# someone-in-somewhere/multimodal_rag

Hardware: AMD Instinct MI355X
Metric: chunks embedded/sec + queries/sec top_k=5 over 1M×768 at 1/2/4/8 GPUs (higher is better)
Workload: dtype f16

## Files before the change

### include/mmrag.h

```cpp
#ifndef MMRAG_H
#define MMRAG_H

#include <stddef.h>
#include <stdint.h>

#ifdef __cplusplus
extern "C" {
#endif

#define MMRAG_OK 0
#define MMRAG_EINVAL 1
#define MMRAG_EWORKSPACE 2
#define MMRAG_EHIP 3
#define MMRAG_EUNSUPPORTED 4

#define MMRAG_F32 0
#define MMRAG_F16 1
#define MMRAG_BF16 2
#define MMRAG_F8E4M3 3

#define MMRAG_MAX_K 20

int mmrag_abi_version(void);
const char *mmrag_last_error(void);

int64_t mmrag_padded_dim(int d, int dtype);

size_t mmrag_cosine_topk_workspace_bytes(int B, int64_t n, int k);

int mmrag_cosine_topk(const void *q, const void *corpus, int B, int64_t n, int d, int64_t ld,
                      int dtype, int k, int64_t row_offset, const uint32_t *alive_bits,
                      float *out_scores, int64_t *out_rows, void *workspace,
                      size_t workspace_bytes, void *stream);

int mmrag_cosine_topk_lists(const void *q, const void *corpus, int B, int64_t n, int d, int64_t ld,
                            int dtype, int k, const uint32_t *alive_bits, void *workspace,
                            size_t workspace_bytes, void *stream);
int mmrag_cosine_topk_select(int B, int64_t n, int k, int64_t row_offset, const void *workspace,
                             float *out_scores, int64_t *out_rows, void *stream);

#define MMRAG_MAX_K_DEEP 4096
size_t mmrag_cosine_topk_deep_workspace_bytes(int B, int64_t n, int k);
int mmrag_cosine_topk_deep(const void *q, const void *corpus, int B, int64_t n, int d, int64_t ld,
                           int dtype, int k, int64_t row_offset, const uint32_t *alive_bits,
                           float *out_scores, int64_t *out_rows, void *workspace,
                           size_t workspace_bytes, void *stream);

#define MMRAG_MAX_RESCORE_CANDIDATES 4096
int mmrag_rescore_topk(const void *q, const void *plane, int64_t ld, int dtype, int d, const int64_t *cand_rows,
                       int B, int C, int k, float *out_scores, int64_t *out_rows, void *stream);

int mmrag_merge_topk(const float *scores, const int64_t *rows, int G, int B, int k_in, int k,
                     float *out_scores, int64_t *out_rows, void *stream);
int mmrag_merge_topk_host(const float *scores, const int64_t *rows, int G, int B, int k_in,
                          int k, float *out_scores, int64_t *out_rows);
int mmrag_merge_topk_host_packed(const void *blocks, int G, int B, int k_in, int k,
                                 float *out_scores, int64_t *out_rows);

int mmrag_append_rows(void *corpus, int64_t capacity, int64_t ld, int dtype, int64_t n_used,
                      const float *new_rows, int64_t m, int d, void *stream);

int mmrag_gather_rows(void *dst, const void *src, int64_t ld, int dtype,
                      const int64_t *keep_rows, int64_t m, void *stream);

int mmrag_fetch_rows_f32(const void *corpus, int64_t ld, int dtype, const int64_t *rows,
                         int64_t m, int d, float *out, void *stream);

int mmrag_copy_to_host_async(void *dst_host, const void *src_dev, size_t bytes, void *stream);


#define MMRAG_ACT_NONE 0
#define MMRAG_ACT_GELU 1
// ... 191 lines not shown
```

### multimodal_rag_amd/_native.py

```python
from __future__ import annotations

import ctypes
import os
import threading
from ctypes import c_char_p, c_float, c_int, c_int32, c_int64, c_size_t, c_void_p
from typing import Optional, Tuple

import numpy as np
import torch

_PKG = os.path.dirname(os.path.abspath(__file__))
LIB_PATH = os.path.join(_PKG, "lib", "libmmrag.so")

F32, F16, BF16, F8E4M3 = 0, 1, 2, 3
MAX_K = 20
MAX_K_DEEP = 4096
MAX_MMR_CANDIDATES = 1024
MAX_RESCORE_CANDIDATES = 4096
MAX_GROUP_CANDIDATES, MAX_GROUPS, MAX_GROUP_SIZE = 4096, 256, 16
MAX_FUSE_LISTS, MAX_FUSE_CANDIDATES, MAX_FUSE_RESULTS = 16, 256, 4096
FUSE_METHODS = {"rrf": 0, "max": 1}
MAX_JOIN_PAIRS = 1 << 26
MAX_CLUSTERS = 4096
MAX_SCOPE_GROUPS = 64
MAX_RELATED_ROWS, MAX_RELATED_SETS = 8192, 64
MAX_RECOMMEND_EXAMPLES = 16
MAX_LATE_QUERY_TOKENS, MAX_LATE_DOC_TOKENS = 128, 512
MAX_LATE_PAIRS = 65535
_DT2TORCH = {F32: torch.float32, F16: torch.float16, BF16: torch.bfloat16, F8E4M3: torch.float8_e4m3fn}
_TORCH2DT = {v: k for k, v in _DT2TORCH.items()}

_lib = None
_lock = threading.Lock()


class MMRagNativeError(RuntimeError):
    pass


def _declare(lib):
    lib.mmrag_abi_version.restype = c_int
    lib.mmrag_last_error.restype = c_char_p
    lib.mmrag_padded_dim.restype = c_int64
    lib.mmrag_padded_dim.argtypes = [c_int, c_int]
    lib.mmrag_cosine_topk_workspace_bytes.restype = c_size_t
    lib.mmrag_cosine_topk_workspace_bytes.argtypes = [c_int, c_int64, c_int]
    lib.mmrag_cosine_topk.restype = c_int
    lib.mmrag_cosine_topk.argtypes = [c_void_p, c_void_p, c_int, c_int64, c_int, c_int64, c_int, c_int,
                                      c_int64, c_void_p, c_void_p, c_void_p, c_void_p, c_size_t, c_void_p]
    lib.mmrag_cosine_topk_lists.restype = c_int
    lib.mmrag_cosine_topk_lists.argtypes = [c_void_p, c_void_p, c_int, c_int64, c_int, c_int64, c_int, c_int,
                                            c_void_p, c_void_p, c_size_t, c_void_p]
    lib.mmrag_internal_search_uses_qs.restype = c_int
    lib.mmrag_internal_search_uses_qs.argtypes = [c_int, c_int64, c_int64, c_int, c_int]
    lib.mmrag_internal_cosine_topk_lists_ex.restype = c_int
    lib.mmrag_internal_cosine_topk_lists_ex.argtypes = [c_void_p, c_void_p, c_int, c_int64, c_int, c_int64, c_int,
                                                        c_int, c_void_p, c_void_p, c_size_t, c_void_p, ctypes.c_uint]
    lib.mmrag_cosine_topk_select.restype = c_int
    lib.mmrag_cosine_topk_select.argtypes = [c_int, c_int64, c_int, c_int64, c_void_p, c_void_p, c_void_p, c_void_p]
    lib.mmrag_cosine_topk_deep_workspace_bytes.restype = c_size_t
    lib.mmrag_cosine_topk_deep_workspace_bytes.argtypes = [c_int, c_int64, c_int]
    lib.mmrag_cosine_topk_deep.restype = c_int
    lib.mmrag_cosine_topk_deep.argtypes = lib.mmrag_cosine_topk.argtypes
    lib.mmrag_internal_cosine_topk_deep_ex.restype = c_int
    lib.mmrag_internal_cosine_topk_deep_ex.argtypes = lib.mmrag_cosine_topk.argtypes + [ctypes.c_uint, c_int64]
    lib.mmrag_rescore_topk.restype = c_int
    lib.mmrag_rescore_topk.argtypes = [c_void_p, c_void_p, c_int64, c_int, c_int, c_void_p, c_int, c_int, c_int,
                                       c_void_p, c_void_p, c_void_p]
    lib.mmrag_merge_topk.restype = c_int
    lib.mmrag_merge_topk.argtypes = [c_void_p, c_void_p, c_int, c_int, c_int, c_int, c_void_p, c_void_p, c_void_p]
    lib.mmrag_merge_topk_host.restype = c_int
    lib.mmrag_merge_topk_host.argtypes = [c_void_p, c_void_p, c_int, c_int, c_int, c_int, c_void_p, c_void_p]
    lib.mmrag_merge_topk_host_packed.restype = c_int
    lib.mmrag_merge_topk_host_packed.argtypes = [c_void_p, c_int, c_int, c_int, c_int, c_void_p, c_void_p]
    lib.mmrag_append_rows.restype = c_int
    lib.mmrag_append_rows.argtypes = [c_void_p, c_int64, c_int64, c_int, c_int64, c_void_p, c_int64, c_int, c_void_p]
    lib.mmrag_gather_rows.restype = c_int
    lib.mmrag_gather_rows.argtypes = [c_void_p, c_void_p, c_int64, c_int, c_void_p, c_int64, c_void_p]
    lib.mmrag_fetch_rows_f32.restype = c_int
    lib.mmrag_fetch_rows_f32.argtypes = [c_void_p, c_int64, c_int, c_void_p, c_int64, c_int, c_void_p, c_void_p]
    lib.mmrag_device_info.restype = c_int
    lib.mmrag_device_info.argtypes = [ctypes.POINTER(c_int), ctypes.POINTER(c_int), ctypes.POINTER(c_int64)]
    lib.mmrag_bench_stream_copy.restype = c_int
    lib.mmrag_bench_stream_copy.argtypes = [c_void_p, c_void_p, c_int64, c_void_p]
    lib.mmrag_bench_mfma_f16.restype = c_int
# ... 204 lines not shown
        raise MMRagNativeError(f"{who}: q and {other} must be contiguous 2-D tensors")
    if q.dtype != rows.dtype or q.shape[1] != rows.shape[1]:
        raise MMRagNativeError(f"{who}: q and {other} must share dtype and padded width")
    if n is not None and n > rows.shape[0]:
        raise MMRagNativeError(f"{who}: n={n} exceeds corpus capacity {rows.shape[0]}")


def _topk_out(B: int, k: int, device, packed: bool = False) -> Tuple[torch.Tensor, torch.Tensor]:
    if not packed:
        return (torch.empty((B, k), dtype=torch.float32, device=device),
                torch.empty((B, k), dtype=torch.int64, device=device))
    buf = torch.empty(B * k * 12, dtype=torch.uint8, device=device)
    return buf[B * k * 8:].view(torch.float32).view(B, k), buf[: B * k * 8].view(torch.int64).view(B, k)


def search_uses_query_stationary(B: int, n: int, d: int, k: int, dtype: torch.dtype) -> bool:
    return bool(lib().mmrag_internal_search_uses_qs(B, n, padded_dim(d, dtype), _TORCH2DT[dtype], k))


def search_kernel_name(B: int, n: int, d: int, k: int, dtype: torch.dtype) -> str:
    v = lib().mmrag_internal_search_uses_qs(B, n, padded_dim(d, dtype), _TORCH2DT[dtype], k)
    return {0: "cosine_topk_kernel (slab-ring)", 1: "cosine_topk_qs_kernel", 2: "cosine_topk_walk_kernel"}[v]


def padded_dim(d: int, dtype: torch.dtype) -> int:
    v = lib().mmrag_padded_dim(int(d), _TORCH2DT[dtype])
    if v < 0:
        raise MMRagNativeError(f"padded_dim: bad arguments d={d} dtype={dtype}")
    return int(v)


DBG_NO_PREPASS, DBG_8_WAVES, DBG_NO_QS, DBG_FORCE_QS = 1, 2, 4, 8
DBG_OLD_QS, DBG_MFMA32, DBG_MFMA16, DBG_NO_DYN, DBG_NO_SEED = 0x10000, 0x20000, 0x40000, 0x80000, 0x100000


def cosine_topk(q: torch.Tensor, corpus: torch.Tensor, n: int, d: int, k: int, row_offset: int = 0,
                alive_bits: Optional[torch.Tensor] = None,
                workspace: Optional[torch.Tensor] = None, dbg: int = 0,
                packed_out: bool = False) -> Tuple[torch.Tensor, torch.Tensor]:
    _dev_check(q, corpus, alive_bits)
    _check_q_rows("cosine_topk", q, corpus, n)
    B, ld = q.shape
    L = lib()
    need = L.mmrag_cosine_topk_workspace_bytes(B, n, k)
    if workspace is None or _nbytes(workspace) < need:
        workspace = torch.empty(max(need, 16), dtype=torch.uint8, device=q.device)
    out_s, out_r = _topk_out(B, k, q.device, packed_out)
    if dbg:
        cosine_topk_lists(q, corpus, n, d, k, workspace, alive_bits=alive_bits, dbg=dbg)
        return cosine_topk_select(B, n, k, row_offset, workspace, out_s, out_r)
    with torch.cuda.device(q.device):
        st = L.mmrag_cosine_topk(q.data_ptr(), corpus.data_ptr(), B, n, d, ld, _TORCH2DT[q.dtype], k, row_offset,
                                 alive_bits.data_ptr() if alive_bits is not None else None,
                                 out_s.data_ptr(), out_r.data_ptr(), workspace.data_ptr(), _nbytes(workspace),
                                 _stream_ptr(q.device))
    _check(st, "mmrag_cosine_topk")
    return out_s, out_r


DEEP_DBG_NO_BOUND = 1


def cosine_topk_deep(q: torch.Tensor, corpus: torch.Tensor, n: int, d: int, k: int, row_offset: int = 0,
                     alive_bits: Optional[torch.Tensor] = None, workspace: Optional[torch.Tensor] = None,
                     dbg: int = 0, cap: int = 0) -> Tuple[torch.Tensor, torch.Tensor]:
    _dev_check(q, corpus, alive_bits)
# ... 1127 lines not shown
        st = lib().mmrag_resize_crop_u8(src.data_ptr(), H, W, src.stride(0), bx.data_ptr(), kx.data_ptr(),
                                        int(kx.shape[1]), by.data_ptr(), ky.data_ptr(), int(ky.shape[1]), out_h, out_w,
                                        y_lo, y_hi, tmp.data_ptr(), out.data_ptr(), _stream_ptr(src.device))
    _check(st, "mmrag_resize_crop_u8")
    return out


def copy_to_host_async(dst_host: torch.Tensor, src_dev: torch.Tensor, stream: int) -> None:
    nbytes = src_dev.numel() * src_dev.element_size()
    if dst_host.is_cuda or not src_dev.is_cuda or dst_host.numel() * dst_host.element_size() < nbytes:
        raise MMRagNativeError("copy_to_host_async: need a host destination at least as large as the device source")
    _check(lib().mmrag_copy_to_host_async(dst_host.data_ptr(), src_dev.data_ptr(), nbytes, stream),
           "mmrag_copy_to_host_async")


class SearchPlan:

    def __init__(self, q: torch.Tensor, corpus: torch.Tensor, n: int, d: int, k: int, workspace: torch.Tensor,
                 alive_bits: Optional[torch.Tensor] = None):
        _dev_check(q, corpus, workspace, alive_bits)
        if q.dtype != corpus.dtype or q.shape[1] != corpus.shape[1] or not q.is_contiguous() or not corpus.is_contiguous():
            raise MMRagNativeError("SearchPlan: q and corpus must be contiguous and share dtype and padded width")
        if n > corpus.shape[0]:
            raise MMRagNativeError(f"SearchPlan: n={n} exceeds corpus capacity {corpus.shape[0]}")
        need = lib().mmrag_cosine_topk_workspace_bytes(q.shape[0], n, k)
        if _nbytes(workspace) < need:
            raise MMRagNativeError("SearchPlan: workspace too small")
        self._keep = (q, corpus, workspace, alive_bits)
        self.B, self.n, self.k = q.shape[0], n, k
        self._scan_args = (q.data_ptr(), corpus.data_ptr(), q.shape[0], n, d, q.shape[1], _TORCH2DT[q.dtype], k,
                           alive_bits.data_ptr() if alive_bits is not None else None, workspace.data_ptr(),
                           _nbytes(workspace))
        self._ws = workspace.data_ptr()
        self._scan = lib().mmrag_cosine_topk_lists
        self._select = lib().mmrag_cosine_topk_select

    def scan(self, stream: int) -> None:
        st = self._scan(*self._scan_args, stream)
        if st:
            _check(st, "mmrag_cosine_topk_lists")

    def select(self, row_offset: int, out_scores_ptr: int, out_rows_ptr: int, stream: int) -> None:
        st = self._select(self.B, self.n, self.k, row_offset, self._ws, out_scores_ptr, out_rows_ptr, stream)
        if st:
            _check(st, "mmrag_cosine_topk_select")
```

### multimodal_rag_amd/csrc/search.hip

```cpp
#include "slab_ring.h"

#include <stdlib.h>

using namespace mmrag;

namespace mmrag_impl {

template <int DT, int WN, int K, int NSTAGE, int NW, bool SEEDED>
__global__ __launch_bounds__(64 * NW, NW / 4) void cosine_topk_kernel(const KParams p) {
#if defined(__HIP_DEVICE_COMPILE__)
#include "slab_ring_body.inc"
#endif
}

template <int K>
struct FullList {
    float v[K];
    long long r[K];
    __device__ inline void init() {
#pragma unroll
        for (int i = 0; i < K; ++i) {
            v[i] = NEG_INF;
            r[i] = LLONG_MAX;
        }
    }
    __device__ inline void insert(float x, long long xr) {
#pragma unroll
        for (int j = 0; j < K; ++j) {
            const bool b = better(x, xr, v[j], r[j]);
            const float nv = b ? x : v[j];
            const float nx = b ? v[j] : x;
            const long long nr = b ? xr : r[j];
            const long long nxr = b ? r[j] : xr;
            v[j] = nv;
            x = nx;
// ... 83 lines not shown
                    out_r[(size_t)q * k_out + i] = valid ? orr[i] + row_offset : -1;
                }
            }
            if (thr0 != nullptr) {
                const bool full = orr[K - 1] != LLONG_MAX && ov[K - 1] > NEG_INF;
                thr0[q] = full ? ov[K - 1] : NEG_INF;
#pragma unroll
                for (int i = 0; i < K; ++i) {
                    const bool valid = orr[i] != LLONG_MAX && ov[i] > NEG_INF;
                    seed_s[(size_t)q * seed_q_stride + i] = valid ? ov[i] : NEG_INF;
                    seed_r[(size_t)q * seed_q_stride + i] = valid ? (int)orr[i] : INT_MAX;
                }
            }
        }
    }
}

struct Plan {
    int K;
    int WN;
    int NW;
    int grid_x, grid_y;
    int n_tiles;
    int n_lists;
    int b_pad;
    int pre_tiles;
    bool qs_ok;
    bool qs_room;
};

constexpr unsigned DBG_NO_PREPASS = 1u, DBG_8_WAVES = 2u, DBG_NO_QS = 4u, DBG_FORCE_QS = 8u;
constexpr unsigned DBG_OLD_QS = 0x10000u, DBG_MFMA32 = 0x20000u, DBG_MFMA16 = 0x40000u, DBG_NO_DYN = 0x80000u,
                   DBG_NO_SEED = 0x100000u;

Plan make_plan(int B, long long n, int k, unsigned dbg = 0) {
    Plan pl;
    pl.K = k <= 5 ? 5 : (k <= 10 ? 10 : 20);
    pl.WN = plan_wn(B);
    const int qrows = 32 * pl.WN;
    pl.grid_y = (B + qrows - 1) / qrows;
    pl.n_tiles = (int)((n + TM - 1) / TM);
    const int cus = num_cus();
    pl.grid_x = plan_walkers(pl.n_tiles, pl.grid_y);
    pl.NW = (pl.K == 5 && pl.WN == 8 && !(dbg & DBG_8_WAVES)) ? 16 : 8;
    pl.pre_tiles = 0;
    const bool want_pre = (pl.WN == 8 || pl.K > 5) && pl.n_tiles >= 3 * cus;
    if (want_pre && !(dbg & DBG_NO_PREPASS)) pl.pre_tiles = cus;
    pl.n_lists = pl.grid_x + (want_pre ? 1 : 0);
    pl.b_pad = pl.grid_y * qrows;
    pl.qs_room = pl.WN == 8 && pl.n_tiles >= cus;
    const bool long_enough = pl.K <= 5 ? pl.n_tiles * 4 >= 15 * cus : pl.n_tiles >= 6 * cus;
    pl.qs_ok = pl.qs_room && !(dbg & DBG_NO_QS) && (long_enough || (dbg & DBG_FORCE_QS));
    return pl;
}

template <int DT, int WN, int K, int NSTAGE, int NW = 8, bool SEEDED = false>
void launch_main(const KParams &p, dim3 grid, hipStream_t s) {
    KParams kp = p;
    kp.walkers = (int)grid.x;
    kp.share_l2 = grid.y > 1;
    cosine_topk_kernel<DT, WN, K, NSTAGE, NW, SEEDED><<<grid.x * grid.y, 64 * NW, 0, s>>>(kp);
}

template <int DT, int K>
void dispatch_deep(const Plan &pl, const KParams &p, dim3 grid, hipStream_t s) {
    if (pl.WN == 2) launch_main<DT, 2, K, 3>(p, grid, s);
// ... 64 lines not shown
__global__ void fill_seed_empty_kernel(float *s, int *r, long long q_stride, int K, long long n_queries) {
    const long long q = (long long)blockIdx.x * blockDim.x + threadIdx.x;
    if (q < n_queries)
        for (int i = 0; i < K; ++i) {
            s[q * q_stride + i] = NEG_INF;
            r[q * q_stride + i] = INT_MAX;
        }
}

int check_search_args(const char *name, int k_max, const void *q, const void *corpus, int B, int64_t n, int d, int64_t ld,
                      int dtype, int k) {
    MMRAG_CHECK_ARG(dtype >= 0 && dtype <= MMRAG_F8E4M3, "%s: bad dtype %d", name, dtype);
    MMRAG_CHECK_ARG(B > 0, "%s: B must be positive (got %d)", name, B);
    MMRAG_CHECK_ARG(k >= 1 && k <= k_max, "%s: k=%d outside 1..%d", name, k, k_max);
    MMRAG_CHECK_ARG(n >= 0 && n < (int64_t)INT_MAX - TM, "%s: n=%lld out of range", name, (long long)n);
    MMRAG_CHECK_ARG(d > 0 && ld >= d, "%s: need 0 < d <= ld (d=%d ld=%lld)", name, d, (long long)ld);
    const int64_t row_bytes = ld * esize(dtype);
    MMRAG_CHECK_ARG(row_bytes % SLAB == 0, "%s: row bytes %lld not a multiple of %d (use mmrag_padded_dim)", name,
                    (long long)row_bytes, SLAB);
    MMRAG_CHECK_ARG(row_bytes * TM < (int64_t)UINT_MAX, "%s: rows too long", name);
    MMRAG_CHECK_ARG(q, "%s: null q", name);
    MMRAG_CHECK_ARG(n == 0 || corpus, "%s: null corpus", name);
    MMRAG_CHECK_ARG(((uintptr_t)q % 16) == 0 && ((uintptr_t)corpus % 16) == 0, "%s: q/corpus must be 16-byte aligned",
                    name);
    return MMRAG_OK;
}

}
using namespace mmrag_impl;

extern "C" {

struct WsLayout {
    size_t entries, off_r, off_thr, off_ts, off_tr, off_cnt, cnt_bytes, off_pub, off_pthr, off_tk, xch_end, total;
};
static WsLayout ws_layout(const Plan &pl) {
    WsLayout w;
    w.entries = (size_t)pl.b_pad * pl.n_lists * pl.K;
    w.off_r = w.entries * sizeof(float);
    w.off_thr = w.off_r + w.entries * sizeof(int);
    w.off_ts = w.off_thr + (size_t)pl.b_pad * sizeof(float);
    w.off_tr = (w.off_ts + (size_t)pl.b_pad * pl.K * sizeof(float) + 15) / 16 * 16;
    w.off_cnt = (w.off_tr + (size_t)pl.b_pad * pl.K * sizeof(long long) + 63) / 64 * 64;
    w.cnt_bytes = 0;
    w.off_pub = w.off_cnt + w.cnt_bytes;
    w.off_pthr = w.off_pub + (pl.qs_room ? (size_t)pl.b_pad * pl.grid_x * sizeof(float) : 0);
    w.off_tk = w.off_pthr + (pl.qs_room ? (size_t)pl.b_pad * sizeof(float) : 0);
    w.xch_end = w.off_tk + (pl.qs_room ? ((size_t)pl.grid_y * sizeof(unsigned) + 63) / 64 * 64 : 0);
    w.total = w.xch_end;
    return w;
}

size_t mmrag_cosine_topk_workspace_bytes(int B, int64_t n, int k) {
    if (B <= 0 || n < 0 || k < 1 || k > MMRAG_MAX_K) return 0;
    return ws_layout(make_plan(B, n, k)).total + 256;
}

int mmrag_internal_cosine_topk_lists_ex(const void *q, const void *corpus, int B, int64_t n, int d, int64_t ld,
                                        int dtype, int k, const uint32_t *alive_bits, void *workspace,
                                        size_t workspace_bytes, void *stream, unsigned dbg) {
    if (int st = check_search_args("cosine_topk", MMRAG_MAX_K, q, corpus, B, n, d, ld, dtype, k)) return st;
    if (n == 0) return MMRAG_OK;
    const Plan pl = make_plan(B, n, k, dbg);
    const WsLayout wl = ws_layout(pl);
    if (!workspace || workspace_bytes < wl.total) {
        set_error("cosine_topk: workspace %zu bytes < required %zu", workspace_bytes, wl.total);
        return MMRAG_EWORKSPACE;
    }
    MMRAG_CHECK_ARG(((uintptr_t)workspace % 16) == 0, "cosine_topk: workspace must be 16-byte aligned");

    KParams p;
    p.q = (const char *)q;
    p.corpus = (const char *)corpus;
    p.alive_bits = alive_bits;
    p.cand_s = (float *)workspace;
    p.cand_r = (int *)((char *)workspace + wl.off_r);
    p.n = n;
    p.B = B;
    p.row_bytes = (unsigned)(ld * esize(dtype));
    p.n_tiles = pl.n_tiles;
    p.n_lists = pl.n_lists;
    p.tile0 = 0;
    p.thr0 = nullptr;
    p.dbg = dbg;
    p.stamps = ((dbg & DBG_QS_CLOCK) && workspace_bytes >= wl.total + 256 * (size_t)(pl.grid_x * pl.grid_y)) ? (unsigned long long *)((char *)workspace + wl.total) : nullptr;
    p.walkers = pl.grid_x;
    p.share_l2 = pl.grid_y > 1;
    p.sample_best = nullptr;
    p.pub_best = nullptr;
    p.pub_thr = nullptr;
    p.tickets = nullptr;
    p.p_static = INT_MAX / 2;
    hipStream_t s = (hipStream_t)stream;
    const size_t seed_off = (size_t)(pl.n_lists - 1) * pl.K;
    const int walk_mfma = (dbg & DBG_MFMA32) ? 32 : ((dbg & DBG_MFMA16) ? 16 : (pl.K == 5 ? QSW_DEFAULT_MFMA : 32));
    if (pl.qs_ok && !(dbg & DBG_OLD_QS) && qsw_supported(dtype, p.row_bytes, pl.K, walk_mfma)) {
        const int tiles = (int)((n + QS_TILE_ROWS - 1) / QS_TILE_ROWS);
        const int per = tiles / pl.grid_x;
        p.n_tiles = tiles;
        p.pub_best = nullptr;
        p.pub_thr = nullptr;
        p.tickets = nullptr;
        p.p_static = INT_MAX / 2;
        const bool seed = per >= 12 && !(dbg & DBG_NO_SEED);
        const bool dyn = pl.grid_y == 1 && per >= 24 && !(dbg & DBG_NO_DYN);
        if (seed || dyn) {
            MMRAG_CHECK_HIP(hipMemsetD32Async((hipDeviceptr_t)((char *)workspace + wl.off_pub), (int)TICKET0,
                                              (wl.xch_end - wl.off_pub) / 4, s));
            if (seed) {
                p.pub_best = (float *)((char *)workspace + wl.off_pub);
                p.pub_thr = (float *)((char *)workspace + wl.off_pthr);
            }
            if (dyn) {
                p.tickets = (unsigned *)((char *)workspace + wl.off_tk);
                const int tail = per / 10 > 3 ? per / 10 : 3;
                p.p_static = per - tail;
            }
        }
        if (int st = qsw_launch(dtype, pl.K, walk_mfma, p, pl.grid_x, pl.grid_y, s)) return st;
        MMRAG_CHECK_HIP(hipGetLastError());
        return MMRAG_OK;
    }
    if (pl.qs_ok && qs_supported(dtype, p.row_bytes, pl.K)) {
        const int tiles = (int)((n + QS_TILE_ROWS - 1) / QS_TILE_ROWS);
        float *thr0 = nullptr;
        if (pl.pre_tiles > 0) {
            KParams ks = p;
            ks.n_tiles = pl.pre_tiles * (TM / QS_TILE_ROWS);
            ks.sample_best = (float *)((char *)workspace + wl.off_pub);
            if (int st = qs_launch(dtype, pl.K, ks, pl.grid_x, pl.grid_y, s)) return st;
            thr0 = (float *)((char *)workspace + wl.off_thr);
            if (int st = qs_seed_thresholds(pl.K, ks.sample_best, pl.grid_x, pl.b_pad, thr0, s)) return st;
        }
        p.n_tiles = tiles;
        p.thr0 = thr0;
        if (int st = qs_launch(dtype, pl.K, p, pl.grid_x, pl.grid_y, s)) return st;
        MMRAG_CHECK_HIP(hipGetLastError());
        return MMRAG_OK;
    }
    auto run = [&](int tile0, int n_tiles, int grid_x, const float *thr0) -> int {
        KParams kp = p;
// ... 16 lines not shown
        const long long n_cand = (long long)pre_grid * pl.K;
        launch_merge<int>(pl.K, p.cand_s, p.cand_r, n_cand, n_cand, 0, (long long)pl.n_lists * pl.K, B, pl.K, 0, top_s,
                          top_r, s, thr0, p.cand_s + seed_off, p.cand_r + seed_off, (long long)pl.n_lists * pl.K);
        MMRAG_CHECK_HIP(hipGetLastError());
        if (int st = run(pre, pl.n_tiles - pre, pl.grid_x, thr0)) return st;
    } else {
        if (pl.n_lists > pl.grid_x) {
            const long long total = (long long)pl.b_pad;
            fill_seed_empty_kernel<<<(unsigned)((total + 255) / 256), 256, 0, s>>>(
                p.cand_s + seed_off, p.cand_r + seed_off, (long long)pl.n_lists * pl.K, pl.K, total);
        }
        if (int st = run(0, pl.n_tiles, pl.grid_x, nullptr)) return st;
    }
    MMRAG_CHECK_HIP(hipGetLastError());
    return MMRAG_OK;
}

int mmrag_internal_search_uses_qs(int B, int64_t n, int64_t ld, int dtype, int k) {
    if (B <= 0 || n <= 0 || k <= 0 || k > MMRAG_MAX_K) return 0;
    const Plan pl = make_plan(B, n, k, 0u);
    const unsigned rb = (unsigned)(ld * esize(dtype));
    if (!pl.qs_ok) return 0;
    if (qsw_supported(dtype, rb, pl.K, QSW_DEFAULT_MFMA)) return 2;
    return qs_supported(dtype, rb, pl.K) ? 1 : 0;
}

int mmrag_cosine_topk_lists(const void *q, const void *corpus, int B, int64_t n, int d, int64_t ld, int dtype,
                            int k, const uint32_t *alive_bits, void *workspace, size_t workspace_bytes,
                            void *stream) {
    return mmrag_internal_cosine_topk_lists_ex(q, corpus, B, n, d, ld, dtype, k, alive_bits, workspace,
                                               workspace_bytes, stream, 0u);
}

int mmrag_cosine_topk_select(int B, int64_t n, int k, int64_t row_offset, const void *workspace,
                             float *out_scores, int64_t *out_rows, void *stream) {
    MMRAG_CHECK_ARG(B > 0 && n >= 0 && k >= 1 && k <= MMRAG_MAX_K, "cosine_topk_select: bad shape");
    MMRAG_CHECK_ARG(out_scores && out_rows, "cosine_topk_select: null output");
    hipStream_t s = (hipStream_t)stream;
    if (n == 0) {
        const long long total = (long long)B * k;
        fill_empty_kernel<<<(unsigned)((total + 255) / 256), 256, 0, s>>>(out_scores, (long long *)out_rows, total);
        MMRAG_CHECK_HIP(hipGetLastError());
        return MMRAG_OK;
    }
    MMRAG_CHECK_ARG(workspace, "cosine_topk_select: null workspace");
    const Plan pl = make_plan(B, n, k);
    const WsLayout wl = ws_layout(pl);
    const float *cand_s = (const float *)workspace;
    const int *cand_r = (const int *)((const char *)workspace + wl.off_r);
    const long long n_cand = (long long)pl.n_lists * pl.K;
    launch_merge<int>(pl.K, cand_s, cand_r, n_cand, n_cand, 0, n_cand, B, k, row_offset, out_scores,
                      (long long *)out_rows, s);
    MMRAG_CHECK_HIP(hipGetLastError());
    return MMRAG_OK;
}

int mmrag_cosine_topk(const void *q, const void *corpus, int B, int64_t n, int d, int64_t ld, int dtype,
                      int k, int64_t row_offset, const uint32_t *alive_bits, float *out_scores,
                      int64_t *out_rows, void *workspace, size_t workspace_bytes, void *stream) {
    if (int st = mmrag_cosine_topk_lists(q, corpus, B, n, d, ld, dtype, k, alive_bits, workspace, workspace_bytes,
                                         stream))
        return st;
    return mmrag_cosine_topk_select(B, n, k, row_offset, workspace, out_scores, out_rows, stream);
}

int mmrag_merge_topk(const float *scores, const int64_t *rows, int G, int B, int k_in, int k,
// ... 13 lines not shown
```

### multimodal_rag_amd/csrc/search_qsw.hip

```cpp
#include "search_shared.h"

#include <type_traits>
#include <utility>

using namespace mmrag;

namespace mmrag_impl {

namespace {

template <typename F, int... I>
__device__ __forceinline__ void static_for_impl(F &&f, std::integer_sequence<int, I...>) {
    (f(std::integral_constant<int, I>{}), ...);
}
template <int N, typename F>
__device__ __forceinline__ void static_for(F &&f) {
    static_for_impl(f, std::make_integer_sequence<int, N>{});
}

constexpr int QSW_XCH = 2048 + 64;
constexpr int qsw_lists_bytes(int K, int MS) { return K * (MS == 32 ? 2 : 4) * QS_QROWS * 8; }

constexpr SlabRing qsw_ring(int NK, int K, int MS) {
#if defined(MMRAG_QSW_RING16)
// ... 119 lines not shown
    static_assert((NST - 1) * PPS <= 56, "vmcnt range");
    static_assert((G - 1) * SLABB + 48 * SLAB + 2048 < 65536, "ds_read immediate offset");
    static_assert(2 * PPS == KSTG, "one piece after every other statement");
    constexpr int LANDT = ((NST - 2) * PPS + 1 + SPT * PPS - 1) / (SPT * PPS);
    static_assert(LANDT >= 1 && LANDT * SPT * PPS - 1 >= (NST - 2) * PPS, "exchange pieces land before they are used");
    static_assert(LOOK <= 6, "ticket slots");

    __shared__ __attribute__((aligned(1024))) char smem[NST * STAGE + LISTS + QSW_XCH];
    float *lists = (float *)(smem + NST * STAGE);
    float *const gather_lds = (float *)(smem + NST * STAGE + LISTS);
    float *const poll_lds = (float *)(smem + NST * STAGE + LISTS + 1024);
    int *const tk_lds = (int *)(smem + NST * STAGE + LISTS + 2048);

    const int tid = threadIdx.x;
    const int lane = tid & 63;
    const int wave = __builtin_amdgcn_readfirstlane(tid >> 6);
    const int ql = lane & (QW - 1);
    const int sub = lane / QW;
    auto dev_dbg = [&](unsigned flag) -> bool {
#if defined(MMRAG_QSW_DEV)
        return (p.dbg & flag) != 0;
#else
        (void)flag;
        return false;
#endif
    };
    const unsigned long long t_entry = (p.dbg & DBG_QS_CLOCK) ? __builtin_amdgcn_s_memrealtime() : 0ull;

    const unsigned RBy = p.row_bytes;
    const int walkers = p.walkers;
    const int bx = (int)blockIdx.x % walkers;
    const int by = (int)blockIdx.x / walkers;
    const int q0 = by * QS_QROWS;
    const int p_static = p.p_static;
    auto pos_tile = [&](int pos) -> int {
        if (pos < p_static) return bx + pos * walkers;
        return p_static * walkers + (int)((unsigned)__builtin_amdgcn_readfirstlane(tk_lds[pos & 7]) - TICKET0);
    };

    unsigned c_off0;
    {
        const int row = (wave * RB) * 8 + (lane >> 3);
        c_off0 = (unsigned)row * RBy + (unsigned)(((lane & 7) ^ ((row >> 1) & 7)) * 16);
    }
    auto c_off = [&](int i) -> unsigned { return i == 0 ? c_off0 : (c_off0 ^ 64u) + 8u * RBy; };
    int is_pos = 0;
    int fill_tile = bx;
    __amdgpu_buffer_rsrc_t fill_rsrc;
    typedef __attribute__((address_space(3))) char *lds_char_t;
    const lds_char_t wave_lds = (lds_char_t)(lds_ptr_t)(smem + wave * (RB * 1024));
    lds_char_t stage_lds = wave_lds;
    auto fill_open = [&]() {
        const bool real = (unsigned)fill_tile < (unsigned)p.n_tiles && !dev_dbg(DBG_QS_NO_DMA);
        const long long row0 = real ? (dev_dbg(DBG_QS_DMA_L2) ? (long long)bx * R : (long long)fill_tile * R) : 0;
        const long long rows_left = p.n - row0;
        const unsigned c_bytes = real ? (unsigned)((rows_left < R ? rows_left : (long long)R) * (long long)RBy) : 0u;
        fill_rsrc = __builtin_amdgcn_make_buffer_rsrc((void *)(p.corpus + (size_t)row0 * RBy), 0, c_bytes, 0x00020000);
    };
    auto next_fill = [&](auto is_sg_c, int buf) {
        constexpr int IS_SG = decltype(is_sg_c)::value;
        if constexpr (IS_SG == 0) {
            if (is_pos != 0) fill_tile = pos_tile(is_pos);
            fill_open();
            ++is_pos;
        }
        stage_lds = wave_lds + buf * STAGE;
        asm volatile("" : "+s"(stage_lds));
// ... 151 lines not shown
                L.insert_strict_flat(valid && sc >= t ? sc : NEG_INF, row_base + row);
                t = fmaxf(t, L.v[K - 1]);
            }
        } else {
            static_for<NGRP>([&](auto gi_c) {
                constexpr int gi = decltype(gi_c)::value;
                const float a0 = score(qb_c, gi_c, 0), a1 = score(qb_c, gi_c, 1);
                const float a2 = score(qb_c, gi_c, 2), a3 = score(qb_c, gi_c, 3);
                if (__builtin_amdgcn_ballot_w64(fmaxf(fmaxf(a0, a1), fmaxf(a2, a3)) >= t) != 0ull) {
#pragma clang loop unroll(disable)
                    for (int i = 0; i < 4; ++i) {
                        const float s = i == 0 ? a0 : (i == 1 ? a1 : (i == 2 ? a2 : a3));
                        const bool pass = s >= t;
                        if (__builtin_amdgcn_ballot_w64(pass) != 0ull) {
                            L.insert_strict(pass ? s : NEG_INF, row_base + grp_row(gi) + i);
                            t = fmaxf(t, L.v[K - 1]);
                        }
                    }
                }
            });
        }
        float u = fmaxf(L.v[K - 1], __shfl_xor(L.v[K - 1], QW));
#pragma unroll
        for (int i = 0; i + 1 < K; ++i) u = fmaxf(u, fminf(L.v[i], __shfl_xor(L.v[K - 2 - i], QW)));
        if constexpr (NSUB == 4) u = fmaxf(u, __shfl_xor(u, 32));
        thr[qb] = fmaxf(t, u);
#pragma unroll
        for (int i = 0; i < K; ++i) {
            lst_v(qb, i) = L.v[i];
            lst_r(qb, i) = L.r[i];
        }
    };

    const bool seeding = p.pub_best != nullptr;
    const int n_resp = (QS_QROWS + walkers - 1) / walkers;
    auto publish_bests = [&](const int ql, const int sub, float *const my_lists) {
        auto lst_v = [&](int qb, int i) -> float & { return my_lists[(qb * 2 * K + i) * QS_QROWS]; };
        float *dst = p.pub_best + ((size_t)by * walkers + bx) * QS_QROWS + wave * 64 + ql;
        static_for<NQB>([&](auto qb_c) {
            constexpr int qb = decltype(qb_c)::value;
            float v = lst_v(qb, 0);
            v = fmaxf(v, __shfl_xor(v, QW));
            if constexpr (NSUB == 4) v = fmaxf(v, __shfl_xor(v, 32));
            if (sub == 0) __hip_atomic_store(dst + qb * QW, v, __ATOMIC_RELAXED, __HIP_MEMORY_SCOPE_AGENT);
        });
    };
    auto gather_issue = [&](int q) {
        const int ln = lane_now();
        const __amdgpu_buffer_rsrc_t rs = __builtin_amdgcn_make_buffer_rsrc(
            (void *)(p.pub_best + (size_t)by * walkers * QS_QROWS), 0, (unsigned)(walkers * QS_QROWS * 4), 0x00020000);
#pragma unroll
        for (int c = 0; c < 4; ++c)
            __builtin_amdgcn_raw_ptr_buffer_load_lds(rs, (lds_ptr_t)((char *)gather_lds + c * 256), 4,
                                                     (unsigned)(((c * 64 + ln) * QS_QROWS + q) * 4), 0, 0, CP_SC1);
    };
    auto compute_thr = [&](int q) {
        const int ln = lane_now();
        float v[4];
#pragma unroll
        for (int c = 0; c < 4; ++c) v[c] = (c * 64 + ln) < walkers ? gather_lds[c * 64 + ln] : NEG_INF;
        const float t = wave_kth_largest<K>(v[0], v[1], v[2], v[3], ln);
        if (ln == 0)
            __hip_atomic_store(p.pub_thr + (size_t)by * QS_QROWS + q, t, __ATOMIC_RELAXED, __HIP_MEMORY_SCOPE_AGENT);
    };
    auto poll_issue = [&]() {
        const __amdgpu_buffer_rsrc_t rs = __builtin_amdgcn_make_buffer_rsrc(
            (void *)(p.pub_thr + (size_t)by * QS_QROWS), 0, QS_QROWS * 4, 0x00020000);
// ... 120 lines not shown
                    const int rel = ti > pub1 ? ti - (pub1 + 1) : ti - 1;
                    const int jc = rel - LANDT, jg = rel;
                    if (jc >= 0 && jc % STEP == 0 && jc / STEP < n_resp && bx + (jc / STEP) * walkers < QS_QROWS)
                        compute_thr(bx + (jc / STEP) * walkers);
                    if (jg >= 0 && jg % STEP == 0 && jg / STEP < n_resp && bx + (jg / STEP) * walkers < QS_QROWS)
                        gather_issue(bx + (jg / STEP) * walkers);
                    if (polled_at(ti)) poll_issue();
                }
            }
            if ((p.dbg & DBG_QS_CLOCK) && p.stamps != nullptr && ti < 28 && wave == 0 && ln == 0)
                p.stamps[32 * blockIdx.x + 4 + ti] = __builtin_amdgcn_s_memrealtime();
            if (want_ticket) {
                wait_vmcnt<SPT * PPS>();
                unsigned long long saved_exec;
                const unsigned slot = (unsigned)(size_t)(lds_ptr_t)(tk_lds + ((ti + LOOK) & 7));
                asm volatile("s_mov_b64 %0, exec\n\t"
                             "s_mov_b64 exec, 1\n\t"
                             "ds_write_b32 %1, %2\n\t"
                             "s_mov_b64 exec, %0"
                             : "=&s"(saved_exec)
                             : "v"(slot), "v"(tkv)
                             : "memory");
            }
            cur_tile = pos_tile(ti + 1);
        }
    }
    const int tid_e = wave * 64 + lane_now();
    if ((p.dbg & DBG_QS_CLOCK) && p.stamps != nullptr && tid_e == 0) {
        p.stamps[32 * blockIdx.x] = __builtin_amdgcn_s_memtime() - t0c;
        p.stamps[32 * blockIdx.x + 1] = __builtin_amdgcn_s_memrealtime() - t0r;
        p.stamps[32 * blockIdx.x + 2] = t0r - t_entry;
        p.stamps[32 * blockIdx.x + 3] = t_entry;
    }
    __syncthreads();
    if (q0 + tid_e < p.B) {
        const int w = tid_e >> 6, qb = (tid_e / QW) & (NQB - 1), c = tid_e & (QW - 1);
        const float *la = lists + w * 64 + c + (qb * 2 * K) * QS_QROWS;
        TopList<K> m;
#pragma unroll
        for (int i = 0; i < K; ++i) {
            m.v[i] = la[i * QS_QROWS];
            m.r[i] = __float_as_int(la[(K + i) * QS_QROWS]);
        }
        for (int s = 1; s < NSUB; ++s) {
            const float *lb = la + s * QW;
            for (int i = 0; i < K; ++i) {
                const float x = lb[i * QS_QROWS];
                const int xr = __float_as_int(lb[(K + i) * QS_QROWS]);
                if (xr == INT_MAX || !better(x, xr, m.v[K - 1], m.r[K - 1])) break;
                m.insert_ordered(x, xr);
            }
        }
        const size_t base = ((size_t)(q0 + tid_e) * p.n_lists + bx) * K;
#pragma unroll
        for (int i = 0; i < K; ++i) {
            p.cand_s[base + i] = m.v[i];
            p.cand_r[base + i] = m.r[i];
        }
        if (bx == 0 && p.n_lists > walkers) {
            const size_t seed = ((size_t)(q0 + tid_e) * p.n_lists + (p.n_lists - 1)) * K;
#pragma unroll
            for (int i = 0; i < K; ++i) {
                p.cand_s[seed + i] = NEG_INF;
                p.cand_r[seed + i] = INT_MAX;
            }
        }
    }
// ... 54 lines not shown
```

### multimodal_rag_amd/csrc/search_shared.h

```cpp
#pragma once
#include "mmrag_internal.h"
#include "tile_dma.h"

#include <limits.h>

namespace mmrag_impl {

constexpr float NEG_INF = -__builtin_inff();

__device__ inline bool better(float s, long long r, float s2, long long r2) {
    return s > s2 || (s == s2 && r < r2);
}

template <int K>
struct TopList {
    float v[K];
    int r[K];
    __device__ inline void init() {
#pragma unroll
        for (int i = 0; i < K; ++i) {
            v[i] = NEG_INF;
            r[i] = INT_MAX;
        }
    }
// ... 34 lines not shown
            v[j] = c[j] ? (c[j - 1] ? v[j - 1] : x) : v[j];
            r[j] = c[j] ? (c[j - 1] ? r[j - 1] : xr) : r[j];
        }
        v[0] = c[0] ? x : v[0];
        r[0] = c[0] ? xr : r[0];
    }
};

struct KParams {
    const char *q;
    const char *corpus;
    const uint32_t *alive_bits;
    float *cand_s;
    int *cand_r;
    long long n;
    int B;
    unsigned row_bytes;
    int n_tiles;
    int n_lists;
    int tile0;
    int walkers;
    int share_l2;
    const float *thr0;
    unsigned dbg;
    unsigned long long *stamps;
    float *sample_best;
    float *pub_best;
    float *pub_thr;
    unsigned *tickets;
    int p_static;
    int tile_stride;
    unsigned *deep_cnt;
    int deep_cap;
};
constexpr unsigned TICKET0 = 0xff800000u;

constexpr unsigned DBG_QS_NO_SELECT = 16u, DBG_QS_NO_DMA = 32u, DBG_QS_NO_BARRIER = 64u, DBG_QS_DMA_L2 = 512u, DBG_QS_NO_WAIT = 1024u;
constexpr unsigned DBG_QS_CLOCK = 256u;

template <int K>
__device__ inline float wave_kth_largest(float a, float b, float c, float d, int lane) {
    auto ce = [](float &x, float &y) {
        const float hi = fmaxf(x, y), lo = fminf(x, y);
        x = hi;
        y = lo;
    };
    ce(a, b);
    ce(c, d);
    ce(a, c);
    ce(b, d);
    ce(b, c);
    float res = NEG_INF;
    for (int r = 0; r < K; ++r) {
        float m = a;
#pragma unroll
        for (int off = 32; off >= 1; off >>= 1) m = fmaxf(m, __shfl_xor(m, off));
        res = m;
        const unsigned long long owners = __builtin_amdgcn_ballot_w64(a == m);
        if (owners != 0ull && lane == (int)__builtin_ctzll(owners)) {
            a = b;
            b = c;
            c = d;
            d = NEG_INF;
        }
    }
    return res;
}

// ... 46 lines not shown
```

Measured before the change: 665,200.

## Self-reset QS exchange buffers in-kernel instead of per-launch memset

Adds a reserved scan entry point, used by the pre-bound search plan, that skips the hipMemsetD32Async on the threshold/ticket exchange region before each query-stationary launch. The kernel now restores its own publish slots to TICKET0 at exit, and the last block to finish (counted with a nonce-tagged atomic) resets the tickets and writes clean markers. If the markers are missing, the launch falls back to fully static scheduling without seeding. The aim is to drop one memset launch per search, at the cost of a cross-block completion protocol whose correctness depends on every block exiting and on memory visibility between launches.

Result: faster. 672,600, median of 6 (+1.1%).

```diff
diff --git a/include/mmrag.h b/include/mmrag.h
--- a/include/mmrag.h
+++ b/include/mmrag.h
@@ -38,6 +38,9 @@
                             size_t workspace_bytes, void *stream);
 int mmrag_cosine_topk_select(int B, int64_t n, int k, int64_t row_offset, const void *workspace,
                              float *out_scores, int64_t *out_rows, void *stream);
+int mmrag_cosine_topk_lists_reserved(const void *q, const void *corpus, int B, int64_t n, int d, int64_t ld,
+                                     int dtype, int k, const uint32_t *alive_bits, void *workspace,
+                                     size_t workspace_bytes, void *stream);
 
 #define MMRAG_MAX_K_DEEP 4096
 size_t mmrag_cosine_topk_deep_workspace_bytes(int B, int64_t n, int k);
diff --git a/multimodal_rag_amd/_native.py b/multimodal_rag_amd/_native.py
--- a/multimodal_rag_amd/_native.py
+++ b/multimodal_rag_amd/_native.py
@@ -51,6 +51,8 @@
     lib.mmrag_cosine_topk_lists.restype = c_int
     lib.mmrag_cosine_topk_lists.argtypes = [c_void_p, c_void_p, c_int, c_int64, c_int, c_int64, c_int, c_int,
                                             c_void_p, c_void_p, c_size_t, c_void_p]
+    lib.mmrag_cosine_topk_lists_reserved.restype = c_int
+    lib.mmrag_cosine_topk_lists_reserved.argtypes = lib.mmrag_cosine_topk_lists.argtypes
     lib.mmrag_internal_search_uses_qs.restype = c_int
     lib.mmrag_internal_search_uses_qs.argtypes = [c_int, c_int64, c_int64, c_int, c_int]
     lib.mmrag_internal_cosine_topk_lists_ex.restype = c_int
@@ -321,6 +323,7 @@
 
 DBG_NO_PREPASS, DBG_8_WAVES, DBG_NO_QS, DBG_FORCE_QS = 1, 2, 4, 8
 DBG_OLD_QS, DBG_MFMA32, DBG_MFMA16, DBG_NO_DYN, DBG_NO_SEED = 0x10000, 0x20000, 0x40000, 0x80000, 0x100000
+DBG_SELF_RESET = 0x400000
 
 
 def cosine_topk(q: torch.Tensor, corpus: torch.Tensor, n: int, d: int, k: int, row_offset: int = 0,
@@ -1514,7 +1517,7 @@
                            alive_bits.data_ptr() if alive_bits is not None else None, workspace.data_ptr(),
                            _nbytes(workspace))
         self._ws = workspace.data_ptr()
-        self._scan = lib().mmrag_cosine_topk_lists
+        self._scan = lib().mmrag_cosine_topk_lists_reserved
         self._select = lib().mmrag_cosine_topk_select
 
     def scan(self, stream: int) -> None:
diff --git a/multimodal_rag_amd/csrc/search.hip b/multimodal_rag_amd/csrc/search.hip
--- a/multimodal_rag_amd/csrc/search.hip
+++ b/multimodal_rag_amd/csrc/search.hip
@@ -1,6 +1,8 @@
 #include "slab_ring.h"
 
 #include <stdlib.h>
+
+#include <atomic>
 
 using namespace mmrag;
 
@@ -150,6 +152,7 @@
 constexpr unsigned DBG_NO_PREPASS = 1u, DBG_8_WAVES = 2u, DBG_NO_QS = 4u, DBG_FORCE_QS = 8u;
 constexpr unsigned DBG_OLD_QS = 0x10000u, DBG_MFMA32 = 0x20000u, DBG_MFMA16 = 0x40000u, DBG_NO_DYN = 0x80000u,
                    DBG_NO_SEED = 0x100000u;
+constexpr unsigned DBG_SELF_RESET = 0x400000u;
 
 Plan make_plan(int B, long long n, int k, unsigned dbg = 0) {
     Plan pl;
@@ -280,7 +283,7 @@
 extern "C" {
 
 struct WsLayout {
-    size_t entries, off_r, off_thr, off_ts, off_tr, off_cnt, cnt_bytes, off_pub, off_pthr, off_tk, xch_end, total;
+    size_t entries, off_r, off_thr, off_ts, off_tr, off_cnt, cnt_bytes, off_pub, off_pthr, off_tk, xch_end, off_state, total;
 };
 static WsLayout ws_layout(const Plan &pl) {
     WsLayout w;
@@ -295,7 +298,8 @@
     w.off_pthr = w.off_pub + (pl.qs_room ? (size_t)pl.b_pad * pl.grid_x * sizeof(float) : 0);
     w.off_tk = w.off_pthr + (pl.qs_room ? (size_t)pl.b_pad * sizeof(float) : 0);
     w.xch_end = w.off_tk + (pl.qs_room ? ((size_t)pl.grid_y * sizeof(unsigned) + 63) / 64 * 64 : 0);
-    w.total = w.xch_end;
+    w.off_state = w.xch_end;
+    w.total = w.off_state + (pl.qs_room ? XCH_STATE_BYTES : 0);
     return w;
 }
 
@@ -353,8 +357,18 @@
         const bool seed = per >= 12 && !(dbg & DBG_NO_SEED);
         const bool dyn = pl.grid_y == 1 && per >= 24 && !(dbg & DBG_NO_DYN);
         if (seed || dyn) {
-            MMRAG_CHECK_HIP(hipMemsetD32Async((hipDeviceptr_t)((char *)workspace + wl.off_pub), (int)TICKET0,
-                                              (wl.xch_end - wl.off_pub) / 4, s));
+            if (!(dbg & DBG_SELF_RESET)) {
+                MMRAG_CHECK_HIP(hipMemsetD32Async((hipDeviceptr_t)((char *)workspace + wl.off_pub), (int)TICKET0,
+                                                  (wl.total - wl.off_pub) / 4, s));
+            } else {
+                static std::atomic<unsigned long long> launches{0};
+                p.xch = (unsigned *)((char *)workspace + wl.off_pub);
+                p.xch_thr_off = (unsigned)((wl.off_pthr - wl.off_pub) / 4);
+                p.xch_tk_off = (unsigned)((wl.off_tk - wl.off_pub) / 4);
+                p.xch_state_off = (unsigned)((wl.off_state - wl.off_pub) / 4);
+                p.xch_mark3 = xch_mark3(pl.grid_x, pl.grid_y);
+                p.xch_nonce = (((launches.fetch_add(1) + 1) * 0x9E3779B97F4A7C15ull) >> 24) | 1ull;
+            }
             if (seed) {
                 p.pub_best = (float *)((char *)workspace + wl.off_pub);
                 p.pub_thr = (float *)((char *)workspace + wl.off_pthr);
@@ -437,6 +451,13 @@
                                                workspace_bytes, stream, 0u);
 }
 
+int mmrag_cosine_topk_lists_reserved(const void *q, const void *corpus, int B, int64_t n, int d, int64_t ld, int dtype,
+                                     int k, const uint32_t *alive_bits, void *workspace, size_t workspace_bytes,
+                                     void *stream) {
+    return mmrag_internal_cosine_topk_lists_ex(q, corpus, B, n, d, ld, dtype, k, alive_bits, workspace,
+                                               workspace_bytes, stream, DBG_SELF_RESET);
+}
+
 int mmrag_cosine_topk_select(int B, int64_t n, int k, int64_t row_offset, const void *workspace,
                              float *out_scores, int64_t *out_rows, void *stream) {
     MMRAG_CHECK_ARG(B > 0 && n >= 0 && k >= 1 && k <= MMRAG_MAX_K, "cosine_topk_select: bad shape");
diff --git a/multimodal_rag_amd/csrc/search_qsw.hip b/multimodal_rag_amd/csrc/search_qsw.hip
--- a/multimodal_rag_amd/csrc/search_qsw.hip
+++ b/multimodal_rag_amd/csrc/search_qsw.hip
@@ -175,7 +175,7 @@
     const int bx = (int)blockIdx.x % walkers;
     const int by = (int)blockIdx.x / walkers;
     const int q0 = by * QS_QROWS;
-    const int p_static = p.p_static;
+    int p_static = p.p_static;
     auto pos_tile = [&](int pos) -> int {
         if (pos < p_static) return bx + pos * walkers;
         return p_static * walkers + (int)((unsigned)__builtin_amdgcn_readfirstlane(tk_lds[pos & 7]) - TICKET0);
@@ -393,7 +393,14 @@
         }
     };
 
-    const bool seeding = p.pub_best != nullptr;
+    bool xch_clean = true;
+    if (p.xch != nullptr) {
+        typedef const __attribute__((address_space(4))) uint32_t *scalar_words_t;
+        const scalar_words_t mk = (scalar_words_t)(p.xch + p.xch_state_off);
+        xch_clean = mk[0] == XCH_MARK0 && mk[1] == XCH_MARK1 && mk[2] == XCH_MARK2 && mk[3] == p.xch_mark3;
+    }
+    if (!xch_clean) p_static = INT_MAX / 2;
+    const bool seeding = p.pub_best != nullptr && xch_clean;
     const int n_resp = (QS_QROWS + walkers - 1) / walkers;
     auto publish_bests = [&](const int ql, const int sub, float *const my_lists) {
         auto lst_v = [&](int qb, int i) -> float & { return my_lists[(qb * 2 * K + i) * QS_QROWS]; };
@@ -580,7 +587,43 @@
         p.stamps[32 * blockIdx.x + 2] = t0r - t_entry;
         p.stamps[32 * blockIdx.x + 3] = t_entry;
     }
+    typedef const __attribute__((address_space(4))) KParams *kparams_t;
+    kparams_t pe = (kparams_t)__builtin_amdgcn_kernarg_segment_ptr();
+    asm volatile("" : "+s"(pe));
+    unsigned *const xch = pe->xch;
+    if (xch != nullptr) {
+        __hip_atomic_store(xch + (size_t)blockIdx.x * QS_QROWS + tid_e, TICKET0, __ATOMIC_RELAXED,
+                           __HIP_MEMORY_SCOPE_AGENT);
+        const int rq = bx + tid_e * pe->walkers;
+        if (rq < QS_QROWS)
+            __hip_atomic_store(xch + pe->xch_thr_off + by * QS_QROWS + rq, TICKET0, __ATOMIC_RELAXED,
+                               __HIP_MEMORY_SCOPE_AGENT);
+    }
     __syncthreads();
+    if (xch != nullptr && tid_e == 0) {
+        XchState *const state = (XchState *)(xch + pe->xch_state_off);
+        const unsigned long long nonce = pe->xch_nonce;
+        typedef const __attribute__((address_space(4))) uint32_t *scalar_words_t;
+        const scalar_words_t mk = (scalar_words_t)state->clean;
+        unsigned long long want;
+        if (mk[0] == XCH_MARK0 && mk[1] == XCH_MARK1 && mk[2] == XCH_MARK2 && mk[3] == pe->xch_mark3) {
+            want = __builtin_amdgcn_atomic_inc64((unsigned long *)&state->done, ~0ul, __ATOMIC_RELAXED, "agent") + 1ull;
+        } else {
+            unsigned long long seen = __hip_atomic_load(&state->done, __ATOMIC_RELAXED, __HIP_MEMORY_SCOPE_AGENT);
+            do want = (seen >> 24) == nonce ? seen + 1 : ((nonce << 24) | 1ull);
+            while (!__hip_atomic_compare_exchange_strong(&state->done, &seen, want, __ATOMIC_RELAXED, __ATOMIC_RELAXED,
+                                                         __HIP_MEMORY_SCOPE_AGENT));
+        }
+        if ((want & 0xffffffull) == (unsigned long long)gridDim.x) {
+            for (unsigned i = pe->xch_tk_off; i < pe->xch_state_off; ++i)
+                __hip_atomic_store(xch + i, TICKET0, __ATOMIC_RELAXED, __HIP_MEMORY_SCOPE_AGENT);
+            __hip_atomic_store(&state->done, 0ull, __ATOMIC_RELAXED, __HIP_MEMORY_SCOPE_AGENT);
+            const unsigned mark[4] = {XCH_MARK0, XCH_MARK1, XCH_MARK2, pe->xch_mark3};
+#pragma unroll
+            for (int i = 0; i < 4; ++i)
+                __hip_atomic_store(&state->clean[i], mark[i], __ATOMIC_RELAXED, __HIP_MEMORY_SCOPE_AGENT);
+        }
+    }
     if (q0 + tid_e < p.B) {
         const int w = tid_e >> 6, qb = (tid_e / QW) & (NQB - 1), c = tid_e & (QW - 1);
         const float *la = lists + w * 64 + c + (qb * 2 * K) * QS_QROWS;
diff --git a/multimodal_rag_amd/csrc/search_shared.h b/multimodal_rag_amd/csrc/search_shared.h
--- a/multimodal_rag_amd/csrc/search_shared.h
+++ b/multimodal_rag_amd/csrc/search_shared.h
@@ -90,8 +90,21 @@
     int tile_stride;
     unsigned *deep_cnt;
     int deep_cap;
+    unsigned *xch = nullptr;
+    unsigned xch_thr_off = 0, xch_tk_off = 0, xch_state_off = 0;
+    unsigned xch_mark3 = 0;
+    unsigned long long xch_nonce = 0;
 };
 constexpr unsigned TICKET0 = 0xff800000u;
+struct XchState {
+    unsigned clean[4];
+    unsigned long long done;
+    unsigned pad[10];
+};
+constexpr size_t XCH_STATE_BYTES = sizeof(XchState);
+static_assert(XCH_STATE_BYTES == 64, "exchange state");
+constexpr unsigned XCH_MARK0 = 0x6d6d7261u, XCH_MARK1 = 0x7158c1eau, XCH_MARK2 = 0x9e3779b9u;
+inline unsigned xch_mark3(int walkers, int groups) { return 0x85ebca6bu ^ ((unsigned)walkers * 0x10001u + (unsigned)groups); }
 
 constexpr unsigned DBG_QS_NO_SELECT = 16u, DBG_QS_NO_DMA = 32u, DBG_QS_NO_BARRIER = 64u, DBG_QS_DMA_L2 = 512u, DBG_QS_NO_WAIT = 1024u;
 constexpr unsigned DBG_QS_CLOCK = 256u;
```
